# ViacheslavDanilov/oct_segmentation

Hardware: AMD Instinct MI355X
Metric: OCT frames/sec (704x704, bf16) fwd+bwd (higher is better)
Workload: dtype bf16; 1 GPU; unetplusplus/resnet101 1-class 704x704, batch 16/GPU, fwd+Dice+bwd+allreduce+Adam; global_batch=16, parallelism=dp1

## Files before the change

oct_segmentation_amd/csrc/gemm1x1.hip:

```cpp
#include "common.h"
#include "conv_common.h"
#include "kernels.h"

#include <cstdlib>
#include <type_traits>

namespace octseg {

constexpr int G1_BM = 128;
constexpr int G1_D = 3;
constexpr int G1_MAXWG = 512;

struct G1Args {
  const char* x; long long xstride;
  const float* scale; const float* shift; int relu;
  const char* w;
  char* y; long long ystride; int accum;
  int M, K, N, n_tiles, m_tiles;
  float* slab; int slab_row0;
  const float* bias; int relu_out;
};

template <typename T, int NT, bool AFF>
__global__ __launch_bounds__(256, 2) void gemm1x1_kernel(const G1Args a) {
  constexpr int D = G1_D;
  constexpr int NSET = D + 1;
  constexpr int NSLOT = 2;
  constexpr int BN = NT * 32;
  constexpr int SLAB = BN * 128;
  constexpr int NPB = SLAB / 4096;
  constexpr int OPITCH = BN * 2 + 16;
  constexpr int PPR = BN / 8;
  constexpr int RPI = 64 / PPR;
  extern __shared__ __attribute__((aligned(16))) char smem[];
  char* ldsB = smem;
  char* strip0 = smem + NSLOT * SLAB;
  float* lds_ss = (float*)(strip0 + 4 * 32 * OPITCH);

  const int tid = threadIdx.x, lane = tid & 63, wave = tid >> 6;
  const int r = lane & 31, h = lane >> 5;
  const int G = gridDim.x;
  const int wid = blockIdx.x;
  const int l = (G & 7) == 0 ? (wid & 7) * (G >> 3) + (wid >> 3) : wid;
  const int nt_idx = l % a.n_tiles, wg_m = l / a.n_tiles, Gm = G / a.n_tiles;
  const int nloc = (a.m_tiles - wg_m + Gm - 1) / Gm;
  const int S = a.K >> 6;
  const int total = nloc * S;
  const int n0 = nt_idx * BN;

  if constexpr (AFF) {
    for (int k = tid; k < a.K; k += 256) { lds_ss[k] = a.scale[k]; lds_ss[a.K + k] = a.shift[k]; }
  }

  int pf_s = 0, pf_mt = wg_m;
  auto row_ptr = [&](int mt) -> const char* {
    const int row = min(mt * G1_BM + wave * 32 + r, a.M - 1);
    return a.x + (long long)row * a.xstride + 64 * h;
  };
  const char* pf_ptr = row_ptr(pf_mt);
  uint4 A[NSET][4];
  auto load_A = [&](uint4 (&dst)[4]) __attribute__((always_inline)) {
#pragma unroll
    for (int j = 0; j < 4; ++j) dst[j] = *(const uint4*)(pf_ptr + 16 * j);
    pf_ptr += 128;
    if (++pf_s == S) {
      pf_s = 0;
      if (pf_mt + Gm < a.m_tiles) pf_mt += Gm;
      pf_ptr = row_ptr(pf_mt);
    }
  };
  int bs = 0;
  const char* wbase = a.w + (long long)nt_idx * SLAB + tid * 16;
  const long long wstep = (long long)a.n_tiles * SLAB;
  uint4 B0 = make_uint4(0, 0, 0, 0), B1 = B0, B2 = B0, B3 = B0;
#define G1_LOAD_B()                                                        \
  do {                                                                     \
    const char* p_ = wbase + bs * wstep;                                   \
    B0 = *(const uint4*)(p_);                                              \
    if constexpr (NPB > 1) B1 = *(const uint4*)(p_ + 4096);                \
    if constexpr (NPB > 2) { B2 = *(const uint4*)(p_ + 8192); B3 = *(const uint4*)(p_ + 12288); } \
    if (++bs == S) bs = 0;                                                 \
  } while (0)
#define G1_STORE_B(slot_)                                                  \
  do {                                                                     \
    char* q_ = ldsB + (slot_) * SLAB + tid * 16;                           \
    *(uint4*)(q_) = B0;                                                    \
    if constexpr (NPB > 1) *(uint4*)(q_ + 4096) = B1;                      \
    if constexpr (NPB > 2) { *(uint4*)(q_ + 8192) = B2; *(uint4*)(q_ + 12288) = B3; } \
  } while (0)

  f32x16_t acc[NT];
#pragma unroll
  for (int nt = 0; nt < NT; ++nt)
#pragma unroll
    for (int v = 0; v < 16; ++v) acc[nt][v] = 0.f;
  float s1[NT], s2[NT];
#pragma unroll
  for (int nt = 0; nt < NT; ++nt) { s1[nt] = 0.f; s2[nt] = 0.f; }

  float obias[NT];
#pragma unroll
  for (int nt = 0; nt < NT; ++nt) obias[nt] = (a.bias != nullptr && n0 + nt * 32 + r < a.N) ? a.bias[n0 + nt * 32 + r] : 0.f;
  const float ofloor = a.relu_out ? 0.f : NO_FLOOR;
  const int bswz = (r >> 1) & 7;
  const int bbase = r * 128;
  const unsigned floor16 = a.relu ? 0u : 0x80008000u;

  G1_LOAD_B();
  G1_STORE_B(0);
  G1_LOAD_B();
#pragma unroll
  for (int d = 0; d < D; ++d) load_A(A[d]);
  __syncthreads();

  int s = 0, mt = wg_m;
  char* strip = strip0 + wave * 32 * OPITCH;

  auto epilogue = [&]() __attribute__((always_inline)) {
    const int m0 = mt * G1_BM + wave * 32;
    if (a.bias != nullptr) {
#pragma unroll
      for (int nt = 0; nt < NT; ++nt)
#pragma unroll
        for (int v = 0; v < 16; ++v) acc[nt][v] = clamp_lo(acc[nt][v] + obias[nt], ofloor);
    }
    if (a.slab != nullptr) {
#pragma unroll
      for (int nt = 0; nt < NT; ++nt)
#pragma unroll
        for (int v = 0; v < 16; ++v) { const float y = acc[nt][v]; s1[nt] += y; s2[nt] += y * y; }
    }
#pragma unroll
    for (int nt = 0; nt < NT; ++nt)
#pragma unroll
      for (int v = 0; v < 16; ++v) {
        const int row = (v & 3) + 8 * (v >> 2) + 4 * h;
        Tr<T>::store(strip + row * OPITCH, nt * 32 + r, acc[nt][v]);
        acc[nt][v] = 0.f;
      }
    __builtin_amdgcn_fence(__ATOMIC_RELEASE, "wavefront");
    asm volatile("s_waitcnt lgkmcnt(0)" ::: "memory");
    const int piece = lane % PPR, rsub = lane / PPR;
    const int n = n0 + piece * 8;
    const bool nok = n < a.N;
    char* gp0 = a.y + (long long)(m0 + rsub) * a.ystride + n * 2;
    const long long gstep = (long long)RPI * a.ystride;
    if (a.accum) {
      uint4 old[32 / RPI];
#pragma unroll
      for (int i = 0; i < 32 / RPI; ++i) {
        const bool ok = nok && m0 + rsub + i * RPI < a.M;
        old[i] = *(const uint4*)(ok ? gp0 + i * gstep : (char*)a.y);
      }
#pragma unroll
      for (int i = 0; i < 32 / RPI; ++i) {
        const int row = rsub + i * RPI;
        if (nok && m0 + row < a.M) {
          const uint4 val = *(const uint4*)(strip + row * OPITCH + piece * 16);
          float x0[8], x1[8];
          Tr<T>::unpack8(val, x0); Tr<T>::unpack8(old[i], x1);
#pragma unroll
          for (int e = 0; e < 8; ++e) x0[e] += x1[e];
          *(uint4*)(gp0 + i * gstep) = Tr<T>::pack8(x0);
        }
      }
    } else {
#pragma unroll
      for (int i = 0; i < 32 / RPI; ++i) {
        const int row = rsub + i * RPI;
        if (nok && m0 + row < a.M) *(uint4*)(gp0 + i * gstep) = *(const uint4*)(strip + row * OPITCH + piece * 16);
      }
    }
    asm volatile("s_waitcnt lgkmcnt(0)" ::: "memory");
  };

  auto step = [&](auto set_c, int g) __attribute__((always_inline)) {
    constexpr int SET = decltype(set_c)::value;
    const int slot = g & 1;
    G1_STORE_B(slot ^ 1);
    G1_LOAD_B();
    load_A(A[(SET + D) % NSET]);
    const bool tail = (mt * G1_BM + G1_BM > a.M);
    const bool valid = mt * G1_BM + wave * 32 + r < a.M;
    const char* bsl = ldsB + slot * SLAB + bbase;
    uint4 bf[2][NT];
#pragma unroll
    for (int nt = 0; nt < NT; ++nt) bf[0][nt] = *(const uint4*)(bsl + nt * 4096 + (((4 * h + 0) ^ bswz) * 16));
#pragma unroll
    for (int j = 0; j < 4; ++j) {
      if (j + 1 < 4) {
#pragma unroll
        for (int nt = 0; nt < NT; ++nt) bf[(j + 1) & 1][nt] = *(const uint4*)(bsl + nt * 4096 + (((4 * h + j + 1) ^ bswz) * 16));
      }
      uint4 af = A[SET][j];
      if constexpr (AFF) {
        const int k0 = s * 64 + 32 * h + 8 * j;
        float sc[8], sh[8];
        const float4 c0 = *(const float4*)(lds_ss + k0), c1 = *(const float4*)(lds_ss + k0 + 4);
        const float4 d0 = *(const float4*)(lds_ss + a.K + k0), d1 = *(const float4*)(lds_ss + a.K + k0 + 4);
        sc[0] = c0.x; sc[1] = c0.y; sc[2] = c0.z; sc[3] = c0.w; sc[4] = c1.x; sc[5] = c1.y; sc[6] = c1.z; sc[7] = c1.w;
        sh[0] = d0.x; sh[1] = d0.y; sh[2] = d0.z; sh[3] = d0.w; sh[4] = d1.x; sh[5] = d1.y; sh[6] = d1.z; sh[7] = d1.w;
        af = Tr<T>::affine_floor(af, sc, sh, floor16);
      }
      if (tail && !valid) af = make_uint4(0, 0, 0, 0);
      __builtin_amdgcn_sched_barrier(0);
#pragma unroll
      for (int nt = 0; nt < NT; ++nt) Tr<T>::mma(af, bf[j & 1][nt], acc[nt]);
      __builtin_amdgcn_sched_barrier(0);
    }
    if (++s == S) {
      epilogue();
      s = 0;
      mt += Gm;
    }
    __syncthreads();
  };

  for (int g = 0; g < total; g += NSET) {
    step(std::integral_constant<int, 0>{}, g);
    if (g + 1 < total) step(std::integral_constant<int, 1>{}, g + 1);
    if (g + 2 < total) step(std::integral_constant<int, 2>{}, g + 2);
    if (g + 3 < total) step(std::integral_constant<int, 3>{}, g + 3);
  }

#undef G1_LOAD_B
#undef G1_STORE_B
  if (a.slab != nullptr) {
    float* red = (float*)strip0;
#pragma unroll
    for (int nt = 0; nt < NT; ++nt) {
      s1[nt] += __shfl_xor(s1[nt], 32);
      s2[nt] += __shfl_xor(s2[nt], 32);
      if (h == 0) { red[(wave * BN + nt * 32 + r) * 2] = s1[nt]; red[(wave * BN + nt * 32 + r) * 2 + 1] = s2[nt]; }
    }
    __syncthreads();
    if (tid < BN && n0 + tid < a.N) {
      float t1 = 0.f, t2 = 0.f;
#pragma unroll
      for (int w = 0; w < 4; ++w) { t1 += red[(w * BN + tid) * 2]; t2 += red[(w * BN + tid) * 2 + 1]; }
      float* o = a.slab + ((size_t)(a.slab_row0 + wg_m) * a.N + n0 + tid) * 2;
      o[0] = t1; o[1] = t2;
    }
  }
}

namespace {

struct G1Geom { int NT, n_tiles, m_tiles, G, rows; size_t lds; };

static G1Geom g1_geom(const ConvArgs& a) {
  G1Geom g;
  g.NT = a.Cout > 64 ? 4 : (a.Cout > 32 ? 2 : 1);
  const int BN = g.NT * 32;
  g.n_tiles = (a.Cout + BN - 1) / BN;
  const long long M = (long long)a.N * a.OH * a.OW;
  g.m_tiles = (int)((M + G1_BM - 1) / G1_BM);
  int gm = G1_MAXWG / g.n_tiles;
  if (gm < 1) gm = 1;
  if (gm > g.m_tiles) gm = g.m_tiles;
  g.rows = gm;
  g.G = gm * g.n_tiles;
  const bool aff = a.src[0].scale != nullptr;
  g.lds = (size_t)2 * BN * 128 + (size_t)4 * 32 * (BN * 2 + 16) + (aff ? (size_t)a.Cin * 8 : 0);
  return g;
}

}

bool gemm1x1_eligible(const ConvArgs& a, int dtype) {
  if (dtype == DT_F32) return false;
  if (a.ntaps != 1 || a.istride != 1 || a.ostride != 1 || a.out_mode == OUT_HEAD_NCHW) return false;
  if (a.tap_dy[0] != 0 || a.tap_dx[0] != 0 || a.nsrc != 1 || a.ndst != 1) return false;
  if (a.bias != nullptr && a.stat_slab != nullptr) return false;
  const SrcDesc& s = a.src[0];
  const DstDesc& d = a.dst[0];
  if (s.up || s.C != a.Cin || s.c0 != 0 || s.H != a.IH || s.W != a.IW || a.IH != a.OH || a.IW != a.OW) return false;
  if (d.pool || d.c0 != 0 || d.H != a.OH || d.W != a.OW || d.cn != a.Cout) return false;
  if (a.Cin % 64 != 0 || a.Cin > 4096 || a.Cout % 8 != 0 || a.Cout < 8) return false;
  if ((long long)a.N * a.OH * a.OW < 1) return false;
  return true;
}

int gemm1x1_rows(const ConvArgs& a) { return g1_geom(a).rows; }

template <typename T, int NT, bool AFF>
static hipError_t g1_launch_k(const G1Args& ga, const G1Geom& g, hipStream_t st) {
  static bool set = false;
  if (!set) {
    hipError_t e = hipFuncSetAttribute((const void*)gemm1x1_kernel<T, NT, AFF>, hipFuncAttributeMaxDynamicSharedMemorySize, 160 * 1024);
    if (e != hipSuccess) return e;
    set = true;
  }
  hipLaunchKernelGGL((gemm1x1_kernel<T, NT, AFF>), dim3(g.G), dim3(256), g.lds, st, ga);
  return hipGetLastError();
}
template <typename T, int NT>
static hipError_t g1_launch(const G1Args& ga, const G1Geom& g, bool aff, hipStream_t st) {
  return aff ? g1_launch_k<T, NT, true>(ga, g, st) : g1_launch_k<T, NT, false>(ga, g, st);
}

hipError_t launch_gemm1x1(int dtype, const ConvArgs& a, hipStream_t st) {
  const G1Geom g = g1_geom(a);
  G1Args ga;
  const SrcDesc& s = a.src[0];
  const DstDesc& d = a.dst[0];
  ga.x = (const char*)s.ptr; ga.xstride = (long long)s.C * 2;
  ga.scale = s.scale; ga.shift = s.shift; ga.relu = s.relu;
  ga.w = (const char*)a.W;
  ga.y = (char*)d.ptr; ga.ystride = (long long)d.C * 2; ga.accum = (d.accum || a.out_mode == OUT_ACCUM) ? 1 : 0;
  ga.M = (int)((long long)a.N * a.OH * a.OW); ga.K = a.Cin; ga.N = a.Cout; ga.n_tiles = g.n_tiles; ga.m_tiles = g.m_tiles;
  ga.slab = a.stat_slab; ga.slab_row0 = a.slab_row0;
  ga.bias = a.bias; ga.relu_out = a.relu_out;
  const bool aff = s.scale != nullptr;
  if (dtype == DT_F16) {
    switch (g.NT) {
      case 4: return g1_launch<f16_t, 4>(ga, g, aff, st);
      case 2: return g1_launch<f16_t, 2>(ga, g, aff, st);
      default: return g1_launch<f16_t, 1>(ga, g, aff, st);
    }
  }
  switch (g.NT) {
    case 4: return g1_launch<bf16_t, 4>(ga, g, aff, st);
    case 2: return g1_launch<bf16_t, 2>(ga, g, aff, st);
    default: return g1_launch<bf16_t, 1>(ga, g, aff, st);
  }
}

}
```

oct_segmentation_amd/csrc/plan_backward.cpp:

```cpp
#include "plan_internal.h"

namespace octseg {
namespace detail {

static int side_wgs() { return 144; }

static int bn_backward(Exec& E, int bn, const void* g, int mask, const void* out_mask, void* res_grad = nullptr, int res_store = 0,
                       const unsigned char* maskbits = nullptr) {
  octseg_plan* P = E.P;
  const BNInfo& b = P->bns[bn];
  const TensorInfo& t = P->tensors[b.y];
  BnBwdArgs a;
  memset(&a, 0, sizeof(a));
  a.g = g; a.y = E.act(b.y); a.out = out_mask; a.maskbits = maskbits;
  a.scale = E.bn_scale(bn); a.shift = E.bn_shift(bn); a.mean = E.bn_mean(bn); a.rstd = E.bn_rstd(bn);
  a.gamma = E.params + P->params[b.gamma].off;
  a.npix = (size_t)t.N * t.H * t.W; a.C = b.C; a.mask = mask;
  a.slab = (float*)(E.ws + P->slab_off);
  a.part = (double*)(E.ws + P->fin_part_off); a.counters = (unsigned*)(E.ws + P->fin_cnt_off);
  const int VEC = P->dtype == DT_F32 ? 4 : 8;
  const int vpc = b.C / VEC;
  const int tpv = vpc >= 256 ? 1 : 256 / vpc;
  size_t rows = (a.npix + tpv - 1) / tpv;
  if (rows > 1024) rows = 1024;
  a.rows = (int)rows;
  a.dgamma = E.grads + P->params[b.gamma].off;
  a.dbeta = E.grads + P->params[b.beta].off;
  a.coef = E.bn_coef(bn);
  a.dy = E.grad(b.y);
  a.res_grad = res_grad; a.res_store = res_store;
  E.ginit[b.y] = 1;
  const double tbytes = (double)a.npix * b.C * dtype_size(P->dtype);
  if (a.npix <= (size_t)BN_SMALL_COUNT) {
    ProfScope ps(3, tbytes * ((mask == 2 && !maskbits) ? 5 : 4), E.st, b.name + ".bwd_small");
    HIPCHK(launch_bn_bwd_small(P->dtype, a, E.st));
    return OCTSEG_OK;
  } else {
    {
      ProfScope ps(3, tbytes * ((mask == 2 && !maskbits) ? 3 : 2), E.st, b.name + ".bwd_reduce");
      HIPCHK(launch_bn_bwd_reduce(P->dtype, a, E.st));
    }
    HIPCHK(launch_bn_bwd_finalize(a, E.st));
  }
  {
    ProfScope ps(3, tbytes * (((mask == 2 && !maskbits) ? 4 : 3) + (res_grad ? (res_store ? 1 : 2) : 0)), E.st, b.name + ".bwd_apply");
    HIPCHK(launch_bn_bwd_apply(P->dtype, a, E.st));
  }
  return OCTSEG_OK;
}

static int conv_backward(Exec& E, const ConvLayer& L, const void* dy, int dyC) {
  octseg_plan* P = E.P;
  const size_t esz = dtype_size(P->dtype);
  const Geom g = E.geom(L);
  if (L.stem && (P->stem_k == 7 && thin_stem_eligible(P->dtype))) {
    if (P->stem_image == nullptr) return fail(OCTSEG_BAD_ARG, "backward without a training forward of this plan (stem frame unknown)");
    hipStream_t ws_ = E.wst ? E.wst : E.st;
    if (ws_ != E.st) {
      HIPCHK(hipEventRecord(P->ev_fork, E.st));
      HIPCHK(hipStreamWaitEvent(ws_, P->ev_fork, 0));
    }
    if (P->dtype == DT_BF16 && !deterministic_mode()) {
      StemArgs sa;
      memset(&sa, 0, sizeof(sa));
      sa.img = P->stem_image; sa.N = P->B; sa.H = P->H; sa.W = P->W; sa.normalize = P->stem_normalize;
      for (int i = 0; i < 3; ++i) { sa.mean[i] = P->stem_mean[i]; sa.stdv[i] = P->stem_std[i]; }
      sa.dy = dy; sa.dW = E.grads + P->params[L.w].off;
      ProfScope ps(2, 2.0 * layer_macs(L), ws_, L.name);
      HIPCHK(launch_thin_stem_wgrad(P->dtype, sa, ws_));
      return OCTSEG_OK;
    }
    const TensorInfo& tc = P->tensors[P->col_tensor];
    HIPCHK(launch_stem_im2col(P->dtype, P->stem_image, E.act(P->col_tensor), P->B, P->H, P->W, tc.C, P->stem_mean, P->stem_std,
                              P->stem_normalize, ws_));
  }
  auto wgrad_part = [&]() -> int {
    hipStream_t ws_ = E.wst ? E.wst : E.st;
    if (ws_ != E.st) {
      HIPCHK(hipEventRecord(P->ev_fork, E.st));
      HIPCHK(hipStreamWaitEvent(ws_, P->ev_fork, 0));
    }
    if (L.b >= 0)
      HIPCHK(launch_channel_sum(P->dtype, dy, (size_t)L.N * L.OH * L.OW, dyC, L.Cout, E.grads + P->params[L.b].off, ws_));
    if (L.tie & 4) {
      SrcDesc src[MAX_SRC];
      const int ns = E.fill_srcs(L, src);
      const int Ca = L.tie_Ca, Cs = L.tie_Cs;
      float* dK4 = (float*)(E.ws + P->tie_scratch_off);
      float* dW3s = dK4 + (size_t)16 * L.Cout * Ca;
      HIPCHK(hipMemsetAsync(dK4, 0, ((size_t)16 * Ca + (size_t)9 * Cs) * L.Cout * sizeof(float), ws_));
      const double macs = layer_macs(L);
      std::vector<WgradArgs> lw;
      wgrad_launches(tie_geom_up(L), lw);
      for (auto& a : lw) {
        a.nsrc = 1; a.src[0] = src[0]; a.src[0].up = 0; a.src[0].c0 = 0;
        a.dy = dy; a.dyC = dyC; a.dW = dK4; a.stamp = nullptr;
        a.wg_target = ws_ != E.st ? side_wgs() : 0;
      }
      if (wgrad_convt16_eligible(lw[0], P->dtype)) {
        ProfScope ps(2, 2.0 * macs * Ca / L.Cin, ws_, L.name);
        HIPCHK(launch_wgrad_convt16(P->dtype, lw[0], ws_));
      } else {
        for (auto& a : lw) {
          ProfScope ps(2, 2.0 * macs * Ca / L.Cin / 4.0, ws_, L.name);
          HIPCHK(launch_wgrad(P->dtype, a, ws_));
        }
      }
      if (Cs > 0) {
        lw.clear();
        wgrad_launches(tie_geom_skip(L), lw);
        WgradArgs& a = lw[0];
        a.nsrc = ns - 1;
        for (int i = 1; i < ns; ++i) { a.src[i - 1] = src[i]; a.src[i - 1].c0 -= Ca; }
        a.dy = dy; a.dyC = dyC; a.dW = dW3s; a.stamp = nullptr;
        a.wg_target = ws_ != E.st ? side_wgs() : 0;
        ProfScope ps(2, 2.0 * macs * Cs / L.Cin, ws_, L.name);
        HIPCHK(launch_wgrad(P->dtype, a, ws_));
      }
      HIPCHK(launch_tied_fold(dK4, Cs > 0 ? dW3s : nullptr, E.grads + P->params[L.w].off, L.Cout, Ca, Cs, ws_));
    } else {
      std::vector<WgradArgs> lw;
      wgrad_launches(g, lw);
      for (auto& a : lw) {
        a.nsrc = E.fill_srcs(L, a.src);
        a.dy = dy; a.dyC = dyC;
        a.dW = E.grads + P->params[L.w].off;
        a.stamp = nullptr;
        a.wg_target = ws_ != E.st ? side_wgs() : 0;
      }
      if (L.transposed && lw.size() == 4 && wgrad_convt16_eligible(lw[0], P->dtype)) {
        ProfScope ps(2, 2.0 * layer_macs(L), ws_, L.name);
        HIPCHK(launch_wgrad_convt16(P->dtype, lw[0], ws_));
        lw.clear();
      }
      const double nl = (double)lw.size();
      for (auto& a : lw) {
        ProfScope ps(2, 2.0 * layer_macs(L) / nl, ws_, L.name);
        HIPCHK(launch_wgrad(P->dtype, a, ws_));
      }
    }
    return OCTSEG_OK;
  };
  auto dgrad_part = [&]() -> int {
    bool any = false;
    for (auto& s : L.srcs) any = any || P->tensors[s.v.t].need_grad;
    if (!any) return OCTSEG_OK;
    if (L.tie & 2) {
      const int ti0 = L.srcs[0].v.t;
      const TensorInfo& t0 = P->tensors[ti0];
      const double macs = layer_macs(L);
      std::vector<ConvArgs> lu;
      if (L.tie_du_masked) { lu.resize(1); tied_dgrad_masked(tie_geom_up(L), lu[0]); }
      else dgrad_launches(tie_geom_up(L), lu);
      const int acc0 = E.claim(ti0);
      for (int k = 0; k < (int)lu.size(); ++k) {
        ConvArgs& a = lu[k];
        if (L.tie_du_masked) {
          for (int p = 0; p < 4; ++p) {
            SrcDesc& s = a.src[p];
            s.ptr = (const char*)dy + ((size_t)(p >> 1) * L.OW + (p & 1)) * dyC * esz;
            s.scale = nullptr; s.shift = nullptr; s.C = 2 * dyC; s.c0 = p * L.Cout; s.H = L.OH / 2; s.W = L.OW; s.up = 0; s.relu = 0;
          }
        } else {
          SrcDesc s;
          s.ptr = dy; s.scale = nullptr; s.shift = nullptr; s.C = dyC; s.c0 = 0; s.H = L.OH; s.W = L.OW; s.up = 0; s.relu = 0;
          a.src[0] = s; a.nsrc = 1;
          a.Cin = L.Cout;
        }
        a.W = E.ws + L.tie_du_off;
        DstDesc d;
        d.ptr = E.grad(ti0); d.C = t0.C; d.c0 = 0; d.cn = L.tie_Ca; d.H = t0.H; d.W = t0.W; d.accum = k == 0 ? acc0 : 1; d.pool = 0;
        a.dst[0] = d; a.ndst = 1; a.out_mode = OUT_STORE; a.bias = nullptr; a.stat_slab = nullptr;
        ProfScope ps(1, 2.0 * macs * L.tie_Ca / L.Cin / (double)lu.size(), E.st, L.name);
        HIPCHK(launch_conv(P->dtype, a, E.st));
      }
      if (L.tie_Cs > 0) {
        std::vector<ConvArgs> ls;
        dgrad_launches(tie_geom_skip(L), ls);
        ConvArgs& a = ls[0];
        SrcDesc s;
        s.ptr = dy; s.scale = nullptr; s.shift = nullptr; s.C = dyC; s.c0 = 0; s.H = L.OH; s.W = L.OW; s.up = 0; s.relu = 0;
        a.src[0] = s; a.nsrc = 1;
        a.Cin = L.Cout;
        a.W = E.ws + L.tie_ds_off;
        int nd = 0, c0 = 0;
        for (size_t i = 1; i < L.srcs.size(); ++i) {
          const int ti = L.srcs[i].v.t;
          const TensorInfo& t = P->tensors[ti];
          DstDesc d;
          d.ptr = E.grad(ti); d.C = t.C; d.c0 = c0; d.cn = t.C; d.H = L.IH; d.W = L.IW; d.accum = E.claim(ti); d.pool = 0;
          a.dst[nd++] = d;
          c0 += t.C;
        }
        a.ndst = nd; a.out_mode = OUT_STORE; a.bias = nullptr; a.stat_slab = nullptr;
        ProfScope ps(1, 2.0 * macs * L.tie_Cs / L.Cin, E.st, L.name);
        HIPCHK(launch_conv(P->dtype, a, E.st));
      }
      return OCTSEG_OK;
    }
    std::vector<ConvArgs> ld;
    dgrad_launches(g, ld);
    bool full_cover = true;
    for (auto& a : ld) if (a.ntaps == 0) full_cover = false;
    DstDesc dst[MAX_SRC];
    int nd = 0, c0 = 0;
    int up_src = -1;
    for (size_t i = 0; i < L.srcs.size(); ++i) {
      const int ti = L.srcs[i].v.t;
      const TensorInfo& t = P->tensors[ti];
      const int scn = L.srcs[i].cn ? L.srcs[i].cn : t.C;
      const size_t soff = (size_t)L.srcs[i].c0 * esz;
      DstDesc d;
      d.C = t.C; d.c0 = c0; d.cn = scn; d.H = L.IH; d.W = L.IW; d.accum = 0; d.pool = 0;
      if (L.srcs[i].up && t.need_grad && ld.size() == 1 && ld[0].ostride == 1 && (L.IH % 2) == 0 && (L.IW % 2) == 0) {
        d.ptr = E.grad(ti); d.H = t.H; d.W = t.W; d.pool = 1;
        d.accum = E.claim(ti);
      } else if (L.srcs[i].up) {
        d.ptr = E.ws + P->tmp_off;
        up_src = (int)i;
      } else if (!t.need_grad) {
        d.ptr = E.ws + P->tmp_off; d.accum = 0;
      } else if (L.srcs[i].cn) {
        if (!E.ginit[ti]) { HIPCHK(hipMemsetAsync(E.grad(ti), 0, (size_t)t.N * t.H * t.W * t.C * esz, E.st)); E.ginit[ti] = 1; }
        d.ptr = (char*)E.grad(ti) + soff;
        d.accum = 1;
      } else {
        d.ptr = E.grad(ti);
        d.accum = E.claim(ti);
        if (!d.accum && !full_cover) {
          HIPCHK(hipMemsetAsync(d.ptr, 0, (size_t)t.N * t.H * t.W * t.C * esz, E.st));
          d.accum = 1;
        }
      }
      dst[nd++] = d;
      c0 += scn;
    }
    for (auto& a : ld) {
      SrcDesc s;
      s.ptr = dy; s.scale = nullptr; s.shift = nullptr; s.C = dyC; s.c0 = 0; s.H = L.OH; s.W = L.OW; s.up = 0; s.relu = 0;
      a.src[0] = s; a.nsrc = 1;
      a.Cin = L.sliced ? L.Cout : dyC;
      a.W = E.ws + L.wimg_dgrad_off;
      if (!L.stem && !L.transposed) { a.Wmaster = E.params + P->params[L.w].off; a.wO = L.Cout; a.wI = L.Cin; a.wtrans = 1; }
      for (int i = 0; i < nd; ++i) a.dst[i] = dst[i];
      a.ndst = nd;
      a.out_mode = OUT_STORE;
      a.bias = nullptr; a.stat_slab = nullptr;
      ProfScope ps(1, 2.0 * layer_macs(L) / (double)ld.size(), E.st, L.name);
      HIPCHK(launch_conv(P->dtype, a, E.st));
    }
    if (up_src >= 0) {
      const TensorInfo& t = P->tensors[L.srcs[up_src].v.t];
      const int ti = L.srcs[up_src].v.t;
      const int acc = E.claim(ti);
      HIPCHK(launch_pool2x2_accum(P->dtype, E.grad(ti), E.ws + P->tmp_off, t.N, t.H, t.W, t.C, acc ? 0 : 1, E.st));
    }
    return OCTSEG_OK;
  };
  { const int rc = wgrad_part(); if (rc) return rc; }
  return dgrad_part();
}

DiceArgs dice_args(const octseg_plan* P, char* ws, const float* logits, const float* target) {
  DiceArgs a;
  memset(&a, 0, sizeof(a));
  a.logits = logits; a.target = target; a.B = P->B; a.C = P->classes; a.HW = (size_t)P->H * P->W;
  a.sums = (double*)(ws + P->dice_off); a.loss_kind = P->loss_kind;
  return a;
}

static void slice_plan(const octseg_plan* P, SliceCtx& S) {
  const int n = S.n;
  S.bounds.assign(n + 1, 0);
  S.bounds[n] = P->param_numel;
  for (int k = 1; k < n; ++k) {
    const size_t want = P->param_numel * (size_t)k / n;
    size_t b = P->param_numel;
    for (auto& q : P->params) if (q.off >= want && q.off < b) b = q.off;
    S.bounds[k] = b;
  }
  for (int k = 1; k <= n; ++k) S.bounds[k] = std::max(S.bounds[k], S.bounds[k - 1]);
  S.last_op.assign(n, -1);
  auto touch = [&](int oi, int param) {
    if (param < 0) return;
    const size_t off = P->params[param].off;
    for (int k = 0; k < n; ++k)
      if (off >= S.bounds[k] && off < S.bounds[k + 1]) { if (S.last_op[k] < 0 || oi < S.last_op[k]) S.last_op[k] = oi; }
  };
  for (int oi = 0; oi < (int)P->ops.size(); ++oi) {
    const Op& op = P->ops[oi];
    if (op.kind == OP_CONV) { touch(oi, P->convs[op.conv].w); touch(oi, P->convs[op.conv].b); }
    else if (op.kind == OP_BN_FIN) { if (P->bns[op.bn].lazy) { touch(oi, P->bns[op.bn].gamma); touch(oi, P->bns[op.bn].beta); } }
    else if (op.kind == OP_GN) { touch(oi, P->gns[op.gn].gamma); touch(oi, P->gns[op.gn].beta); }
    else if (op.kind == OP_DW || op.kind == OP_DWG) touch(oi, op.dwp);
    else if (op.kind == OP_BNX) { touch(oi, P->bns[op.y.bn].gamma); touch(oi, P->bns[op.y.bn].beta); }
    else if (op.kind == OP_SEFC) { for (int i = 0; i < 4; ++i) touch(oi, op.ins[i]); }
    else if (op.kind == OP_FPA) {
      for (int l = 0; l < 6; ++l) { touch(oi, P->fpa.w[l]); touch(oi, P->fpa.b[l]); touch(oi, P->bns[P->fpa.bn[l]].gamma); touch(oi, P->bns[P->fpa.bn[l]].beta); }
    }
    else if (op.kind == OP_BN_ACT) {
      touch(oi, P->bns[op.y.bn].gamma); touch(oi, P->bns[op.y.bn].beta);
      if (op.res.t >= 0 && op.res.bn >= 0) { touch(oi, P->bns[op.res.bn].gamma); touch(oi, P->bns[op.res.bn].beta); }
    }
  }
}

int run_backward(Exec& E, const float* logits, const float* target, float grad_scale, SliceCtx* S) {
  octseg_plan* P = E.P;
  if (S) slice_plan(P, *S);
  auto fire = [&](int k) -> int {
    if (S->bounds[k + 1] == S->bounds[k]) return OCTSEG_OK;
    if (!P->ev_slice) HIPCHK(hipEventCreateWithFlags(&P->ev_slice, hipEventDisableTiming));
    HIPCHK(hipEventRecord(P->ev_slice, E.st));
    HIPCHK(hipStreamWaitEvent(S->comm, P->ev_slice, 0));
    if (E.wst && E.wst != E.st) {
      HIPCHK(hipEventRecord(P->ev_slice, E.wst));
      HIPCHK(hipStreamWaitEvent(S->comm, P->ev_slice, 0));
    }
    S->cb(S->user, k, S->bounds[k], S->bounds[k + 1]);
    return OCTSEG_OK;
  };
  HIPCHK(hipMemsetAsync(E.grads, 0, P->param_numel * sizeof(float), E.st));
  HIPCHK(hipMemsetAsync(E.ws + P->fin_cnt_off, 0, 2 * 64 * sizeof(unsigned), E.st));
  E.ginit.assign(P->tensors.size(), 0);
  if (!serial_mode()) {
    hipStream_t* wsp = P->tgraph_enabled ? &P->side : &P->side_bwd;
    if (!*wsp) HIPCHK(create_side_stream(wsp, !P->tgraph_enabled));
    if (!P->ev_fork) {
      HIPCHK(hipEventCreateWithFlags(&P->ev_fork, hipEventDisableTiming));
      HIPCHK(hipEventCreateWithFlags(&P->ev_join, hipEventDisableTiming));
    }
    E.wst = *wsp;
    HIPCHK(hipEventRecord(P->ev_fork, E.st));
    HIPCHK(hipStreamWaitEvent(E.wst, P->ev_fork, 0));
  }
  const DiceArgs da = dice_args(P, E.ws, logits, target);
  HIPCHK(launch_dice_bwd(P->dtype, da, grad_scale, E.ws + P->dlogits_off, P->dlogits_C, E.st));
  int rc;
  for (int oi = (int)P->ops.size() - 1; oi >= 0; --oi) {
    const Op& op = P->ops[oi];
    switch (op.kind) {
      case OP_STEM_COL: break;
      case OP_CONV: {
        const ConvLayer& L = P->convs[op.conv];
        if (L.head) rc = conv_backward(E, L, E.ws + (P->head_up > 1 ? P->dz4_off : P->dlogits_off), P->dlogits_C);
        else if (L.sliced) rc = conv_backward(E, L, (char*)E.grad(L.out) + (size_t)L.out_c0 * dtype_size(P->dtype), P->tensors[L.out].C);
        else rc = conv_backward(E, L, E.grad(L.out), L.Cout);
        if (rc) return rc;
        break;
      }
      case OP_BN_FIN: {
        const BNInfo& b = P->bns[op.bn];
        if (b.lazy) {
          rc = bn_backward(E, op.bn, E.grad(b.y), 1, nullptr);
          if (rc) return rc;
        }
        break;
      }
      case OP_BN_ACT: {
        const TensorInfo& t = P->tensors[op.out];
        const void* G = E.grad(op.out);
        const size_t n = (size_t)t.N * t.H * t.W * t.C;
        const int mask = !op.relu ? 0 : (op.post >= 0 ? 1 : 2);
        const bool fuse_res = mask == 2 && op.res.t >= 0 && op.res.bn < 0 && P->tensors[op.res.t].need_grad &&
                              E.grad(op.res.t) != G && E.grad(op.res.t) != E.grad(P->bns[op.y.bn].y);
        const unsigned char* mbits = (mask == 2 && t.mask_off) ? (const unsigned char*)(E.ws + t.mask_off) : nullptr;
        if (fuse_res) {
          const int acc = E.claim(op.res.t);
          rc = bn_backward(E, op.y.bn, G, mask, E.act(op.out), E.grad(op.res.t), acc ? 0 : 1, mbits);
        } else {
          rc = bn_backward(E, op.y.bn, G, mask, E.act(op.out), nullptr, 0, mbits);
        }
        if (rc) return rc;
        if (op.res.t >= 0 && !fuse_res) {
          if (op.res.bn >= 0) {
            rc = bn_backward(E, op.res.bn, G, op.relu ? 2 : 0, E.act(op.out), nullptr, 0, (op.relu && t.mask_off) ? (const unsigned char*)(E.ws + t.mask_off) : nullptr);
            if (rc) return rc;
          } else if (P->tensors[op.res.t].need_grad) {
            const int acc = E.claim(op.res.t);
            HIPCHK(launch_masked_accum(P->dtype, E.grad(op.res.t), G, op.relu ? E.act(op.out) : nullptr, n, acc ? 0 : 1, E.st));
          }
        }
        if (op.post >= 0 && P->tensors[op.post].need_grad) {
          const int acc = E.claim(op.post);
          HIPCHK(launch_masked_accum(P->dtype, E.grad(op.post), G, nullptr, n, acc ? 0 : 1, E.st));
        }
        break;
      }
      case OP_DROP2D: {
        const TensorInfo& t = P->tensors[op.out];
        HIPCHK(launch_drop_bwd(P->dtype, E.grad(op.out), P->dropout_keep, 1.0f / (1.0f - P->dropout_p), E.grad(op.in), t.N, (size_t)t.H * t.W, t.C, E.st));
        E.ginit[op.in] = 1;
        break;
      }
      case OP_RELU: {
        const TensorInfo& t = P->tensors[op.out];
        HIPCHK(launch_relu(P->dtype, E.grad(op.out), E.act(op.out), E.grad(op.in), (size_t)t.N * t.H * t.W * t.C, E.st));
        E.ginit[op.in] = 1;
        break;
      }
      case OP_RESIZE: {
        const TensorInfo& ti = P->tensors[op.in];
        const TensorInfo& to = P->tensors[op.out];
        HIPCHK(launch_bilinear_resize_adjoint(P->dtype, E.grad(op.out), E.grad(op.in), ti.N, ti.H, ti.W, to.H, to.W, ti.C, E.st));
        E.ginit[op.in] = 1;
        break;
      }
      case OP_STATS: break;
      case OP_DWG: {
        const TensorInfo& ti = P->tensors[op.in];
        const TensorInfo& to = P->tensors[op.out];
        DwgArgs a;
        memset(&a, 0, sizeof(a));
        a.in = E.act(op.in); a.out = E.grad(op.out); a.w = E.params + P->params[op.dwp].off; a.dw = E.grads + P->params[op.dwp].off;
        a.N = ti.N; a.H = ti.H; a.W = ti.W; a.C = ti.C; a.OH = to.H; a.OW = to.W; a.K = op.wc0; a.stride = op.up; a.pad = op.oc0;
        HIPCHK(launch_dwg_bwd_w(P->dtype, a, E.st));
        if (ti.need_grad) {
          a.gin = E.grad(op.in); a.accum = E.claim(op.in);
          HIPCHK(launch_dwg_bwd_data(P->dtype, a, E.st));
        }
        break;
      }
      case OP_BNX: {
        const TensorInfo& t = P->tensors[op.out];
        BnxArgs a;
        memset(&a, 0, sizeof(a));
        a.y = E.act(op.y.t); a.scale = E.bn_scale(op.y.bn); a.shift = E.bn_shift(op.y.bn);
        a.dscale = op.oc0 >= 0 ? P->drop_connect + (size_t)op.oc0 * t.N : nullptr;
        a.post = E.grad(op.out); a.out = E.grad(op.y.t);
        a.npix = (size_t)t.N * t.H * t.W; a.hw = t.H * t.W; a.C = t.C; a.act = op.up;
        HIPCHK(launch_bnx_bwd(P->dtype, a, E.st));
        rc = bn_backward(E, op.y.bn, E.grad(op.y.t), 0, nullptr);
        if (rc) return rc;
        if (op.post >= 0 && P->tensors[op.post].need_grad) {
          const int acc = E.claim(op.post);
          HIPCHK(launch_masked_accum(P->dtype, E.grad(op.post), E.grad(op.out), nullptr, (size_t)t.N * t.H * t.W * t.C, acc ? 0 : 1, E.st));
        }
        break;
      }
      case OP_SEFC: {
        const TensorInfo& t = P->tensors[op.in];
        SefcArgs a;
        memset(&a, 0, sizeof(a));
        a.m = E.act(op.in); a.ds = E.grad(op.out); a.dm = E.grad(op.in);
        a.w1 = E.params + P->params[op.ins[0]].off; a.w2 = E.params + P->params[op.ins[2]].off;
        a.dw1 = E.grads + P->params[op.ins[0]].off; a.db1 = E.grads + P->params[op.ins[1]].off;
        a.dw2 = E.grads + P->params[op.ins[2]].off; a.db2 = E.grads + P->params[op.ins[3]].off;
        a.h = (float*)(E.ws + op.aux_off); a.dh = a.h + (size_t)t.N * op.up;
        a.N = t.N; a.C = t.C; a.R = op.up; a.act = op.oc0;
        HIPCHK(launch_sefc_bwd(P->dtype, a, E.st));
        E.ginit[op.in] = 1;
        break;
      }
      case OP_SEGATE: {
        const TensorInfo& t = P->tensors[op.in];
        const bool two = op.ins[1] >= 0;
        HIPCHK(launch_se_dgate(P->dtype, E.grad(op.out), E.act(op.in), E.act(op.ins[0]), E.grad(op.ins[0]), (float*)(E.ws + P->se_part_off), t.N, t.H * t.W,
                               t.C, E.st, two ? E.act(op.ins[1]) : nullptr, two ? E.grad(op.ins[1]) : nullptr));
        E.ginit[op.ins[0]] = 1;
        if (two) E.ginit[op.ins[1]] = 1;
        const int acc = E.claim(op.in);
        HIPCHK(launch_se_gate(P->dtype, E.grad(op.out), E.act(op.ins[0]), E.grad(op.in), t.N, t.H * t.W, t.C, acc, E.st, two ? E.act(op.ins[1]) : nullptr));
        break;
      }
      case OP_ADD: {
        const TensorInfo& t = P->tensors[op.out];
        const size_t n = (size_t)t.N * t.H * t.W * t.C;
        for (int src : {op.in, op.ins[0]})
          if (P->tensors[src].need_grad) {
            const int acc = E.claim(src);
            HIPCHK(launch_masked_accum(P->dtype, E.grad(src), E.grad(op.out), nullptr, n, acc ? 0 : 1, E.st));
          }
        break;
      }
      case OP_FPA: {
        const TensorInfo& t = P->tensors[op.in];
        const int n1 = t.N * (t.H / 2) * (t.W / 2);
        float* scr = (float*)(E.ws + P->fpa.scratch_off);
        float* gs = (float*)(E.ws + P->fpa.gscratch_off);
        float* duu = gs + fpa_pyr_gscratch_floats(t.N, t.H, t.W);
        HIPCHK(launch_fpa_mix(P->dtype, scr + fpa_pyr_uu_offset(t.N, t.H, t.W), E.act(op.ins[0]), nullptr, nullptr, E.grad(op.out), E.grad(op.ins[0]), duu, t.N,
                              t.H * t.W, 32, E.st));
        E.ginit[op.ins[0]] = 1;
        HIPCHK(launch_image_sum(P->dtype, E.grad(op.out), E.grad(op.ins[1]), t.N, t.H * t.W, 32, 1.f, E.st));
        E.ginit[op.ins[1]] = 1;
        FpaPyrArgs a;
        memset(&a, 0, sizeof(a));
        a.N = t.N; a.h = t.H; a.w = t.W; a.train = 1; a.scratch = scr; a.gscratch = gs; a.duu = duu;
        for (int l = 0; l < 6; ++l) {
          const BNInfo& bn = P->bns[P->fpa.bn[l]];
          a.w_[l] = E.params + P->params[P->fpa.w[l]].off; a.b_[l] = E.params + P->params[P->fpa.b[l]].off;
          a.g_[l] = E.params + P->params[bn.gamma].off; a.be_[l] = E.params + P->params[bn.beta].off;
          a.rm_[l] = E.buffers; a.rv_[l] = E.buffers;
          a.dw_[l] = E.grads + P->params[P->fpa.w[l]].off; a.db_[l] = E.grads + P->params[P->fpa.b[l]].off;
          a.dg_[l] = E.grads + P->params[bn.gamma].off; a.dbe_[l] = E.grads + P->params[bn.beta].off;
        }
        HIPCHK(launch_fpa_pyr_bwd(a, E.st));
        HIPCHK(launch_fpa_in_bwd(P->dtype, E.act(P->fpa.pool), gs + n1, E.params + P->params[P->fpa.w[0]].off, E.grad(P->fpa.pool),
                                 E.grads + P->params[P->fpa.w[0]].off, E.grads + P->params[P->fpa.b[0]].off, t.N, t.H / 2, t.W / 2, t.C, 7, E.st));
        {
          const int acc = E.claim(op.in);
          HIPCHK(launch_maxpool2(P->dtype, E.act(op.in), nullptr, E.grad(P->fpa.pool), E.grad(op.in), t.N, t.H, t.W, t.C, acc, E.st));
        }
        break;
      }
      case OP_PAB: {
        const TensorInfo& t = P->tensors[op.in];
        const int hw = t.H * t.W;
        const size_t sbytes = align_up((size_t)t.N * hw * hw * sizeof(float));
        float* Pm = (float*)(E.ws + op.aux_off);
        float* dP = (float*)(E.ws + op.aux_off + sbytes);
        float* dM = (float*)(E.ws + op.aux_off + 2 * sbytes);
        {
          const int acc = E.claim(op.in);
          HIPCHK(launch_masked_accum(P->dtype, E.grad(op.in), E.grad(op.out), nullptr, (size_t)t.N * hw * t.C, acc ? 0 : 1, E.st));
        }
        HIPCHK(launch_pab_mix(P->dtype, nullptr, nullptr, nullptr, dM, E.grad(op.out), t.N, hw, t.C, E.st));
        PabGemm g;
        memset(&g, 0, sizeof(g));
        g.batch = t.N;
        g.A = dM; g.a_f32 = 1; g.sAb = (size_t)hw * t.C; g.sAm = t.C; g.sAk = 1;
        g.B = E.act(op.ins[2]); g.sBb = (size_t)hw * t.C; g.sBk = 1; g.sBn = t.C;
        g.C = dP; g.c_f32 = 1; g.sCb = (size_t)hw * hw; g.sCm = hw; g.sCn = 1; g.M = hw; g.N = hw; g.K = t.C;
        HIPCHK(launch_pab_gemm(P->dtype, g, E.st));
        g.A = Pm; g.a_f32 = 1; g.sAb = (size_t)hw * hw; g.sAm = 1; g.sAk = hw;
        g.B = dM; g.b_f32 = 1; g.sBb = (size_t)hw * t.C; g.sBk = t.C; g.sBn = 1;
        g.C = E.grad(op.ins[2]); g.c_f32 = 0; g.sCb = (size_t)hw * t.C; g.sCm = t.C; g.sCn = 1; g.M = hw; g.N = t.C; g.K = hw;
        HIPCHK(launch_pab_gemm(P->dtype, g, E.st));
        E.ginit[op.ins[2]] = 1;
        HIPCHK(launch_pab_softmax(dP, Pm, t.N, (size_t)hw * hw, 1, E.st));
        g.A = dP; g.a_f32 = 1; g.sAb = (size_t)hw * hw; g.sAm = hw; g.sAk = 1;
        g.B = E.act(op.ins[0]); g.b_f32 = 0; g.sBb = (size_t)hw * 64; g.sBk = 64; g.sBn = 1;
        g.C = E.grad(op.ins[1]); g.sCb = (size_t)hw * 64; g.sCm = 64; g.sCn = 1; g.M = hw; g.N = 64; g.K = hw;
        HIPCHK(launch_pab_gemm(P->dtype, g, E.st));
        E.ginit[op.ins[1]] = 1;
        g.sAm = 1; g.sAk = hw;
        g.B = E.act(op.ins[1]);
        g.C = E.grad(op.ins[0]);
        HIPCHK(launch_pab_gemm(P->dtype, g, E.st));
        E.ginit[op.ins[0]] = 1;
        break;
      }
      case OP_MOSAIC: {
        const TensorInfo& tf = P->tensors[op.oc0 ? op.in : op.out];
        const int acc = E.claim(op.in);
        HIPCHK(launch_mosaic(P->dtype, E.grad(op.out), E.grad(op.in), tf.N, tf.H, tf.W, tf.C, op.up, op.oc0 ? 0 : 1, op.oc0 ? acc : 0, E.st));
        break;
      }
      case OP_BINPOOL: {
        const TensorInfo& t = P->tensors[op.in];
        const int acc = E.claim(op.in);
        HIPCHK(launch_bin_mean_bwd(P->dtype, E.grad(op.out), E.grad(op.in), t.N, t.H, t.W, t.C, op.up, acc, E.st));
        break;
      }
      case OP_UPB: {
        const TensorInfo& t = P->tensors[op.in];
        HIPCHK(launch_bilinear_adjoint(P->dtype, E.grad(op.out), E.grad(op.in), t.N, t.H, t.W, t.C, op.up, E.st));
        E.ginit[op.in] = 1;
        break;
      }
      case OP_DROPE: {
        const TensorInfo& t = P->tensors[op.out];
        HIPCHK(launch_drop_elem(P->dtype, E.grad(op.out), P->dropout_keep, 1.0f / (1.0f - P->dropout_p), E.grad(op.in),
                                (size_t)t.N * t.H * t.W * t.C, E.st));
        E.ginit[op.in] = 1;
        break;
      }
      case OP_BCAST: {
        const TensorInfo& t = P->tensors[op.out];
        HIPCHK(launch_image_sum(P->dtype, E.grad(op.out), E.grad(op.in), t.N, t.H * t.W, t.C, 1.f, E.st));
        E.ginit[op.in] = 1;
        break;
      }
      case OP_GAP: {
        const TensorInfo& t = P->tensors[op.in];
        const int acc = E.claim(op.in);
        HIPCHK(launch_image_bcast(P->dtype, E.grad(op.out), E.grad(op.in), t.N, t.H * t.W, t.C, 1.f / (float)(t.H * t.W), acc, E.st));
        break;
      }
      case OP_DW: {
        const TensorInfo& ti = P->tensors[op.in];
        const TensorInfo& to = P->tensors[op.out];
        const ParamInfo& w = P->params[op.dwp];
        HIPCHK(launch_dw_wgrad(P->dtype, E.act(op.in), ti.C, 0, E.grad(op.out), to.C, op.oc0, E.grads + w.off, w.O, op.wc0, ti.N, ti.H, ti.W, ti.C,
                               op.up, E.st));
        if (ti.need_grad) {
          const int acc = E.claim(op.in);
          HIPCHK(launch_dw_conv(P->dtype, E.grad(op.out), to.C, op.oc0, E.grad(op.in), ti.C, 0, E.params + w.off, w.O, op.wc0, ti.N, ti.H, ti.W,
                                ti.C, op.up, 1, acc, E.st));
        }
        break;
      }
      case OP_PARITY: {
        const TensorInfo& tf = P->tensors[op.up ? op.in : op.out];
        const int acc = E.claim(op.in);
        HIPCHK(launch_parity_permute(P->dtype, E.grad(op.out), E.grad(op.in), tf.N, tf.H, tf.W, tf.C, op.up ? 0 : 1, acc, E.st));
        break;
      }
      case OP_UPLOGITS: {
        const int h4 = P->H / P->head_up, w4 = P->W / P->head_up;
        HIPCHK(launch_bilinear_adjoint(P->dtype, E.ws + P->dlogits_off, E.ws + P->dz4_off, P->B, h4, w4, P->dlogits_C, P->head_up, E.st));
        break;
      }
      case OP_MERGE: {
        const TensorInfo& t = P->tensors[op.out];
        HIPCHK(launch_drop_bwd(P->dtype, E.grad(op.out), P->dropout_keep, 1.0f / (1.0f - P->dropout_p), E.grad(op.ins[0]), t.N, (size_t)t.H * t.W,
                               t.C, E.st));
        for (int i = 0; i < 4; ++i) E.ginit[op.ins[i]] = 1;
        break;
      }
      case OP_GN: {
        const TensorInfo& t = P->tensors[op.in];
        GnArgs ga = E.gn_args(op.gn);
        if (op.up > 1) {
          HIPCHK(launch_bilinear_adjoint(P->dtype, E.grad(op.out), E.grad(op.in), t.N, t.H, t.W, t.C, op.up, E.st));
          ga.g = E.grad(op.in);
        } else {
          ga.g = E.grad(op.out);
        }
        ga.dy = E.grad(op.in);
        E.ginit[op.in] = 1;
        HIPCHK(launch_gn_backward(P->dtype, ga, t.N, E.st));
        break;
      }
      case OP_UP2: {
        const TensorInfo& t = P->tensors[op.in];
        const int acc = E.claim(op.in);
        HIPCHK(launch_pool2x2_accum(P->dtype, E.grad(op.in), E.grad(op.out), t.N, t.H, t.W, t.C, acc ? 0 : 1, E.st));
        break;
      }
      case OP_MAXPOOL: {
        const TensorInfo& t = P->tensors[op.in];
        const int acc = E.claim(op.in);
        HIPCHK(launch_maxpool_bwd_idx(P->dtype, (const unsigned char*)(E.ws + P->pool_idx_off), E.grad(op.out), E.grad(op.in), t.N, t.H, t.W,
                                      t.C, acc ? 0 : 1, E.st));
        break;
      }
    }
    if (S)
      for (int k = 0; k < S->n; ++k)
        if (S->last_op[k] == oi) { rc = fire(k); if (rc) return rc; }
  }
  if (S)
    for (int k = 0; k < S->n; ++k)
      if (S->last_op[k] < 0) { rc = fire(k); if (rc) return rc; }
  if (E.wst && E.wst != E.st) {
    HIPCHK(hipEventRecord(P->ev_join, E.wst));
    HIPCHK(hipStreamWaitEvent(E.st, P->ev_join, 0));
  }
  return OCTSEG_OK;
}

}
}
```

Measured before the change: 254.5 frames/s.

## Deepen 1x1 GEMM weight prefetch, specialize accumulate path, skip empty dgrad launches

The 1x1 GEMM kernel now keeps two alternating register sets for weight-tile prefetch (P/Q), so the global load for tile g+2 is issued while tile g+1 is being stored to LDS. Sched barriers separate the LDS store from the next global load, and the prologue is reordered to interleave A and B loads. The accumulate mode becomes a template parameter and the main loop's per-step bounds checks are removed, with the epilogue guarded instead. Separately, dgrad launches for decomposed sub-convolutions with zero taps are skipped. This raises register pressure and assumes that running steps past `total` is harmless.

New measurement: 254.1 frames/s (median of 2 runs). About the same (-0.2%).

```diff
diff --git a/oct_segmentation_amd/csrc/gemm1x1.hip b/oct_segmentation_amd/csrc/gemm1x1.hip
--- a/oct_segmentation_amd/csrc/gemm1x1.hip
+++ b/oct_segmentation_amd/csrc/gemm1x1.hip
@@ -15,13 +15,13 @@
   const char* x; long long xstride;
   const float* scale; const float* shift; int relu;
   const char* w;
-  char* y; long long ystride; int accum;
+  char* y; long long ystride;
   int M, K, N, n_tiles, m_tiles;
   float* slab; int slab_row0;
   const float* bias; int relu_out;
 };
 
-template <typename T, int NT, bool AFF>
+template <typename T, int NT, bool AFF, bool ACC>
 __global__ __launch_bounds__(256, 2) void gemm1x1_kernel(const G1Args a) {
   constexpr int D = G1_D;
   constexpr int NSET = D + 1;
@@ -72,21 +72,21 @@
   int bs = 0;
   const char* wbase = a.w + (long long)nt_idx * SLAB + tid * 16;
   const long long wstep = (long long)a.n_tiles * SLAB;
-  uint4 B0 = make_uint4(0, 0, 0, 0), B1 = B0, B2 = B0, B3 = B0;
-#define G1_LOAD_B()                                                        \
+  uint4 P0 = make_uint4(0, 0, 0, 0), P1 = P0, P2 = P0, P3 = P0, Q0 = P0, Q1 = P0, Q2 = P0, Q3 = P0;
+#define G1_LOAD_B(R)                                                       \
   do {                                                                     \
     const char* p_ = wbase + bs * wstep;                                   \
-    B0 = *(const uint4*)(p_);                                              \
-    if constexpr (NPB > 1) B1 = *(const uint4*)(p_ + 4096);                \
-    if constexpr (NPB > 2) { B2 = *(const uint4*)(p_ + 8192); B3 = *(const uint4*)(p_ + 12288); } \
+    R##0 = *(const uint4*)(p_);                                            \
+    if constexpr (NPB > 1) R##1 = *(const uint4*)(p_ + 4096);              \
+    if constexpr (NPB > 2) { R##2 = *(const uint4*)(p_ + 8192); R##3 = *(const uint4*)(p_ + 12288); } \
     if (++bs == S) bs = 0;                                                 \
   } while (0)
-#define G1_STORE_B(slot_)                                                  \
+#define G1_STORE_B(R, slot_)                                               \
   do {                                                                     \
     char* q_ = ldsB + (slot_) * SLAB + tid * 16;                           \
-    *(uint4*)(q_) = B0;                                                    \
-    if constexpr (NPB > 1) *(uint4*)(q_ + 4096) = B1;                      \
-    if constexpr (NPB > 2) { *(uint4*)(q_ + 8192) = B2; *(uint4*)(q_ + 12288) = B3; } \
+    *(uint4*)(q_) = R##0;                                                  \
+    if constexpr (NPB > 1) *(uint4*)(q_ + 4096) = R##1;                    \
+    if constexpr (NPB > 2) { *(uint4*)(q_ + 8192) = R##2; *(uint4*)(q_ + 12288) = R##3; } \
   } while (0)
 
   f32x16_t acc[NT];
@@ -106,11 +106,14 @@
   const int bbase = r * 128;
   const unsigned floor16 = a.relu ? 0u : 0x80008000u;
 
-  G1_LOAD_B();
-  G1_STORE_B(0);
-  G1_LOAD_B();
-#pragma unroll
-  for (int d = 0; d < D; ++d) load_A(A[d]);
+  load_A(A[0]);
+  uint4 T0 = P0, T1 = P0, T2 = P0, T3 = P0;
+  G1_LOAD_B(T);
+  G1_LOAD_B(P);
+  G1_LOAD_B(Q);
+#pragma unroll
+  for (int d = 1; d < D; ++d) load_A(A[d]);
+  G1_STORE_B(T, 0);
   __syncthreads();
 
   int s = 0, mt = wg_m;
@@ -140,12 +143,14 @@
       }
     __builtin_amdgcn_fence(__ATOMIC_RELEASE, "wavefront");
     asm volatile("s_waitcnt lgkmcnt(0)" ::: "memory");
-    const int piece = lane % PPR, rsub = lane / PPR;
+    int elane = lane;
+    asm volatile("" : "+v"(elane));
+    const int piece = elane % PPR, rsub = elane / PPR;
     const int n = n0 + piece * 8;
     const bool nok = n < a.N;
     char* gp0 = a.y + (long long)(m0 + rsub) * a.ystride + n * 2;
     const long long gstep = (long long)RPI * a.ystride;
-    if (a.accum) {
+    if constexpr (ACC) {
       uint4 old[32 / RPI];
 #pragma unroll
       for (int i = 0; i < 32 / RPI; ++i) {
@@ -177,8 +182,8 @@
   auto step = [&](auto set_c, int g) __attribute__((always_inline)) {
     constexpr int SET = decltype(set_c)::value;
     const int slot = g & 1;
-    G1_STORE_B(slot ^ 1);
-    G1_LOAD_B();
+    if constexpr ((SET & 1) == 0) { G1_STORE_B(P, slot ^ 1); __builtin_amdgcn_sched_barrier(0); G1_LOAD_B(P); }
+    else { G1_STORE_B(Q, slot ^ 1); __builtin_amdgcn_sched_barrier(0); G1_LOAD_B(Q); }
     load_A(A[(SET + D) % NSET]);
     const bool tail = (mt * G1_BM + G1_BM > a.M);
     const bool valid = mt * G1_BM + wave * 32 + r < a.M;
@@ -209,7 +214,7 @@
       __builtin_amdgcn_sched_barrier(0);
     }
     if (++s == S) {
-      epilogue();
+      if (g < total) epilogue();
       s = 0;
       mt += Gm;
     }
@@ -218,9 +223,9 @@
 
   for (int g = 0; g < total; g += NSET) {
     step(std::integral_constant<int, 0>{}, g);
-    if (g + 1 < total) step(std::integral_constant<int, 1>{}, g + 1);
-    if (g + 2 < total) step(std::integral_constant<int, 2>{}, g + 2);
-    if (g + 3 < total) step(std::integral_constant<int, 3>{}, g + 3);
+    step(std::integral_constant<int, 1>{}, g + 1);
+    step(std::integral_constant<int, 2>{}, g + 2);
+    step(std::integral_constant<int, 3>{}, g + 3);
   }
 
 #undef G1_LOAD_B
@@ -283,20 +288,21 @@
 
 int gemm1x1_rows(const ConvArgs& a) { return g1_geom(a).rows; }
 
-template <typename T, int NT, bool AFF>
+template <typename T, int NT, bool AFF, bool ACC>
 static hipError_t g1_launch_k(const G1Args& ga, const G1Geom& g, hipStream_t st) {
   static bool set = false;
   if (!set) {
-    hipError_t e = hipFuncSetAttribute((const void*)gemm1x1_kernel<T, NT, AFF>, hipFuncAttributeMaxDynamicSharedMemorySize, 160 * 1024);
+    hipError_t e = hipFuncSetAttribute((const void*)gemm1x1_kernel<T, NT, AFF, ACC>, hipFuncAttributeMaxDynamicSharedMemorySize, 160 * 1024);
     if (e != hipSuccess) return e;
     set = true;
   }
-  hipLaunchKernelGGL((gemm1x1_kernel<T, NT, AFF>), dim3(g.G), dim3(256), g.lds, st, ga);
+  hipLaunchKernelGGL((gemm1x1_kernel<T, NT, AFF, ACC>), dim3(g.G), dim3(256), g.lds, st, ga);
   return hipGetLastError();
 }
 template <typename T, int NT>
-static hipError_t g1_launch(const G1Args& ga, const G1Geom& g, bool aff, hipStream_t st) {
-  return aff ? g1_launch_k<T, NT, true>(ga, g, st) : g1_launch_k<T, NT, false>(ga, g, st);
+static hipError_t g1_launch(const G1Args& ga, const G1Geom& g, bool aff, bool acc, hipStream_t st) {
+  if (acc) return aff ? g1_launch_k<T, NT, true, true>(ga, g, st) : g1_launch_k<T, NT, false, true>(ga, g, st);
+  return aff ? g1_launch_k<T, NT, true, false>(ga, g, st) : g1_launch_k<T, NT, false, false>(ga, g, st);
 }
 
 hipError_t launch_gemm1x1(int dtype, const ConvArgs& a, hipStream_t st) {
@@ -307,23 +313,24 @@
   ga.x = (const char*)s.ptr; ga.xstride = (long long)s.C * 2;
   ga.scale = s.scale; ga.shift = s.shift; ga.relu = s.relu;
   ga.w = (const char*)a.W;
-  ga.y = (char*)d.ptr; ga.ystride = (long long)d.C * 2; ga.accum = (d.accum || a.out_mode == OUT_ACCUM) ? 1 : 0;
+  ga.y = (char*)d.ptr; ga.ystride = (long long)d.C * 2;
   ga.M = (int)((long long)a.N * a.OH * a.OW); ga.K = a.Cin; ga.N = a.Cout; ga.n_tiles = g.n_tiles; ga.m_tiles = g.m_tiles;
   ga.slab = a.stat_slab; ga.slab_row0 = a.slab_row0;
   ga.bias = a.bias; ga.relu_out = a.relu_out;
   const bool aff = s.scale != nullptr;
+  const bool acc = d.accum || a.out_mode == OUT_ACCUM;
   if (dtype == DT_F16) {
     switch (g.NT) {
-      case 4: return g1_launch<f16_t, 4>(ga, g, aff, st);
-      case 2: return g1_launch<f16_t, 2>(ga, g, aff, st);
-      default: return g1_launch<f16_t, 1>(ga, g, aff, st);
+      case 4: return g1_launch<f16_t, 4>(ga, g, aff, acc, st);
+      case 2: return g1_launch<f16_t, 2>(ga, g, aff, acc, st);
+      default: return g1_launch<f16_t, 1>(ga, g, aff, acc, st);
     }
   }
   switch (g.NT) {
-    case 4: return g1_launch<bf16_t, 4>(ga, g, aff, st);
-    case 2: return g1_launch<bf16_t, 2>(ga, g, aff, st);
-    default: return g1_launch<bf16_t, 1>(ga, g, aff, st);
-  }
-}
-
-}
+    case 4: return g1_launch<bf16_t, 4>(ga, g, aff, acc, st);
+    case 2: return g1_launch<bf16_t, 2>(ga, g, aff, acc, st);
+    default: return g1_launch<bf16_t, 1>(ga, g, aff, acc, st);
+  }
+}
+
+}
diff --git a/oct_segmentation_amd/csrc/plan_backward.cpp b/oct_segmentation_amd/csrc/plan_backward.cpp
--- a/oct_segmentation_amd/csrc/plan_backward.cpp
+++ b/oct_segmentation_amd/csrc/plan_backward.cpp
@@ -235,7 +235,10 @@
       dst[nd++] = d;
       c0 += scn;
     }
+    size_t nlive = 0;
+    for (auto& a : ld) nlive += a.ntaps > 0 ? 1 : 0;
     for (auto& a : ld) {
+      if (a.ntaps == 0) continue;
       SrcDesc s;
       s.ptr = dy; s.scale = nullptr; s.shift = nullptr; s.C = dyC; s.c0 = 0; s.H = L.OH; s.W = L.OW; s.up = 0; s.relu = 0;
       a.src[0] = s; a.nsrc = 1;
@@ -246,7 +249,7 @@
       a.ndst = nd;
       a.out_mode = OUT_STORE;
       a.bias = nullptr; a.stat_slab = nullptr;
-      ProfScope ps(1, 2.0 * layer_macs(L) / (double)ld.size(), E.st, L.name);
+      ProfScope ps(1, 2.0 * layer_macs(L) / (double)nlive, E.st, L.name);
       HIPCHK(launch_conv(P->dtype, a, E.st));
     }
     if (up_src >= 0) {
```
